# tlroy/thermalporous

Measured on AMD Instinct MI355X. Metric: Newton steps/s, SPE10 60x220x85 two-phase (FGMRES its/s in config), higher is better.
Workload: dtype f64; 1 GPU; BASELINE config 4: two-phase 3D SPE10-like 60x220x85, wells+heaters, pc_cptr, maxdt 0.1 day; grid 60x220x85 (synthetic default_rng(10) field); FGMRES rtol 1e-08; timed at dt = maxdt after an untimed spin-up along the reference's dt ramp; newton_its=84, fgmres_its=2692, failed_solves=0, slabs=none

## Files before the change

thermalporous_amd/csrc/tp_amg.hip:

```cpp
#include "tp_common.hpp"
#include <algorithm>
#include <cstdlib>

namespace tp {

template <class R>
struct StencilT {
    R *base;
    long slot_stride;
    __host__ __device__ const R *slot(int s) const { return base + (long)s * slot_stride; }
};

__device__ __forceinline__ void cell_ijk(const GridDev &g, long tid, int &i0, int &i1, int &i2) {
    const unsigned t = (unsigned)tid, np = (unsigned)g.np, n0 = (unsigned)g.n0;
    const unsigned q2 = t / np, rem = t - q2 * np, q1 = rem / n0;
    i2 = (int)q2;
    i1 = (int)q1;
    i0 = (int)(rem - q1 * n0);
}

template <class R>
__global__ void k_amg_weights(GridDev g, StencilT<R> A, int axis, double omega, R *wm, R *wp, R *invd,
                              unsigned long long *ratio_slots) {
    const long tid = (long)blockIdx.x * blockDim.x + threadIdx.x;
// ... 84 lines not shown
        const double piv = M[(long)p * n + p];
        __syncthreads();
        for (int e = threadIdx.x; e < n; e += blockDim.x) {
            M[(long)p * n + e] /= piv;
            Minv[(long)p * n + e] /= piv;
        }
        __syncthreads();
        for (int e = threadIdx.x; e < n * n; e += blockDim.x) {
            const int r = e / n, q = e % n;
            if (r == p) continue;
            const double fct = M[(long)r * n + p];
            Minv[(long)r * n + q] -= fct * Minv[(long)p * n + q];
            if (q != p) M[(long)r * n + q] -= fct * M[(long)p * n + q];
        }
        __syncthreads();
        for (int r = threadIdx.x; r < n; r += blockDim.x)
            if (r != p) M[(long)r * n + p] = 0.0;
        __syncthreads();
    }
}

template <class R>
__global__ __launch_bounds__(1024) void k_amg_dense_inverse_lds(GridDev g, StencilT<R> A, int n, double *Minv_out) {
    __shared__ double M[64 * 64];
    __shared__ double I[64 * 64];
    __shared__ double col[64];
    const int t = threadIdx.x, T = blockDim.x;
    const long off[7] = {0, -1, 1, -(long)g.n0, (long)g.n0, -g.np, g.np};
    for (int e = t; e < 64 * 64; e += T) { M[e] = 0.0; I[e] = ((e >> 6) == (e & 63)) ? 1.0 : 0.0; }
    __syncthreads();
    for (int r = t; r < n; r += T) {
        const long c = g.np + r;
        int i0, i1, i2;
        cell_ijk(g, r, i0, i1, i2);
        const bool has[7] = {true, i0 > 0, i0 < g.n0 - 1, i1 > 0, i1 < g.n1 - 1, i2 > 0, i2 < g.n2 - 1};
        for (int s = 0; s < 7; ++s)
            if (has[s]) M[r * 64 + (int)(r + off[s])] += (double)A.slot(s)[c];
    }
    __syncthreads();
    for (int p = 0; p < n; ++p) {
        if (t < n) col[t] = M[t * 64 + p];
        __syncthreads();
        const double piv = col[p];
        if (t < n) M[p * 64 + t] /= piv;
        else if (t >= 64 && t < 64 + n) I[p * 64 + (t - 64)] /= piv;
        __syncthreads();
        for (int e = t; e < n * 64; e += T) {
            const int r = e >> 6, q = e & 63;
            if (r == p || q >= n) continue;
            const double fct = col[r];
            I[e] -= fct * I[p * 64 + q];
            M[e] = (q == p) ? 0.0 : M[e] - fct * M[p * 64 + q];
        }
        __syncthreads();
    }
    for (int e = t; e < n * n; e += T) Minv_out[e] = I[(e / n) * 64 + e % n];
}

typedef double mfma_d4 __attribute__((ext_vector_type(4)));
template <class R>
__global__ __launch_bounds__(1024) void k_amg_dense_inverse_mfma(GridDev g, StencilT<R> A, int n, double *Minv_out) {
    extern __shared__ double lds[];
    double *X = lds;
    double *Rb = X + 64 * 128;
    double *Cb = Rb + 4 * 128;
    double *Pi = Cb + 64 * 4;
    const int t = threadIdx.x, T = blockDim.x, lane = t & 63, wave = t >> 6;
    const long off[7] = {0, -1, 1, -(long)g.n0, (long)g.n0, -g.np, g.np};
    for (int e = t; e < 64 * 128; e += T) {
        const int r = e >> 7, q = e & 127;
        X[e] = (q == r + 64 || (q == r && r >= n)) ? 1.0 : 0.0;
    }
    __syncthreads();
    for (int r = t; r < n; r += T) {
        const long c = g.np + r;
        int i0, i1, i2;
        cell_ijk(g, r, i0, i1, i2);
        const bool has[7] = {true, i0 > 0, i0 < g.n0 - 1, i1 > 0, i1 < g.n1 - 1, i2 > 0, i2 < g.n2 - 1};
        for (int s = 0; s < 7; ++s)
            if (has[s]) X[r * 128 + (int)(r + off[s])] += (double)A.slot(s)[c];
    }
    __syncthreads();
    for (int p0 = 0; p0 < 64; p0 += 4) {
        if (t == 0) {
            double P[4][4], Q[4][4];
#pragma unroll
            for (int i = 0; i < 4; ++i)
#pragma unroll
                for (int j = 0; j < 4; ++j) { P[i][j] = X[(p0 + i) * 128 + p0 + j]; Q[i][j] = i == j ? 1.0 : 0.0; }
#pragma unroll
            for (int p = 0; p < 4; ++p) {
                const double ip = 1.0 / P[p][p];
#pragma unroll
                for (int j = 0; j < 4; ++j) { P[p][j] *= ip; Q[p][j] *= ip; }
#pragma unroll
                for (int i = 0; i < 4; ++i) {
                    if (i == p) continue;
                    const double f = P[i][p];
#pragma unroll
                    for (int j = 0; j < 4; ++j) { P[i][j] -= f * P[p][j]; Q[i][j] -= f * Q[p][j]; }
                }
            }
#pragma unroll
            for (int i = 0; i < 4; ++i)
#pragma unroll
                for (int j = 0; j < 4; ++j) Pi[i * 4 + j] = Q[i][j];
        }
        __syncthreads();
        if (t < 512) {
            const int i = t >> 7, q = t & 127;
            double v = 0.0;
#pragma unroll
            for (int m = 0; m < 4; ++m) v += Pi[i * 4 + m] * X[(p0 + m) * 128 + q];
            Rb[i * 128 + q] = v;
        } else if (t < 768) {
            const int r = (t - 512) >> 2, j = t & 3;
            Cb[r * 4 + j] = (r >= p0 && r < p0 + 4) ? 0.0 : X[r * 128 + p0 + j];
        }
        __syncthreads();
#pragma unroll
        for (int h = 0; h < 2; ++h) {
            const int rt = wave >> 2, ct = 2 * (wave & 3) + h;
            const double a = -Cb[(rt * 16 + (lane & 15)) * 4 + (lane >> 4)];
            const double b = Rb[(lane >> 4) * 128 + ct * 16 + (lane & 15)];
            mfma_d4 acc;
            double *xp = X + (rt * 16 + (lane >> 4)) * 128 + ct * 16 + (lane & 15);
#pragma unroll
            for (int q = 0; q < 4; ++q) acc[q] = xp[q * 4 * 128];
            acc = __builtin_amdgcn_mfma_f64_16x16x4f64(a, b, acc, 0, 0, 0);
#pragma unroll
            for (int q = 0; q < 4; ++q) {
                const int row = rt * 16 + (lane >> 4) + 4 * q;
                xp[q * 4 * 128] = (row >= p0 && row < p0 + 4) ? Rb[(row - p0) * 128 + ct * 16 + (lane & 15)] : acc[q];
            }
        }
        __syncthreads();
    }
    for (int e = t; e < n * n; e += T) Minv_out[e] = X[(e / n) * 128 + 64 + e % n];
}

template <class R>
struct LevelDevT {
    GridDev g;
    StencilT<R> op;
    const R *invd, *wm, *wp;
    double *b, *x, *x2, *e;
    int axis;
    int pre, post;
    int pad_;
    double omega;
};

template <class R, bool REG>
__device__ __forceinline__ double invd_at(const LevelDevT<R> &L, long c) {
    if constexpr (REG) return (double)(R)(L.omega / (double)L.op.slot(0)[c]);
    else return (double)L.invd[c];
}

__device__ __forceinline__ void nb_offsets(const GridDev &g, long (&off)[7]) {
    off[0] = 0; off[1] = -1; off[2] = 1; off[3] = -(long)g.n0; off[4] = g.n0; off[5] = -g.np; off[6] = g.np;
}

template <class R, bool REG>
__device__ __forceinline__ double pre2_cell(const LevelDevT<R> &L, const double *__restrict__ b, long tid) {
    const long c = L.g.np + tid;
    long off[7];
    nb_offsets(L.g, off);
    double s = 0.0, ic = 0.0;
#pragma unroll
    for (int k = 0; k < 7; ++k) {
        const long n = c + off[k];
        double iv;
        if constexpr (REG) {
            const double d = (double)L.op.slot(0)[n];
            const double q = (double)(R)(L.omega / d);
            iv = d != 0.0 ? q : 0.0;
        } else {
            iv = (double)L.invd[n];
        }
        if (k == 0) ic = iv;
        s += L.op.slot(k)[c] * (iv * b[n]);
    }
    const double x1 = ic * b[c];
    return x1 + ic * (b[c] - s);
}

template <class R, bool REG = false>
__device__ __forceinline__ double jacobi_cell(const LevelDevT<R> &L, const double *__restrict__ b,
                                              const double *__restrict__ x, long tid) {
    const long c = L.g.np + tid;
    long off[7];
    nb_offsets(L.g, off);
    double s = 0.0;
#pragma unroll
    for (int k = 0; k < 7; ++k) s += L.op.slot(k)[c] * x[c + off[k]];
    return x[c] + invd_at<R, REG>(L, c) * (b[c] - s);
}

template <class R>
__device__ __forceinline__ double resid_at(const LevelDevT<R> &L, const double *__restrict__ b,
                                           const double *__restrict__ x, long c) {
    long off[7];
    nb_offsets(L.g, off);
    double s = 0.0;
#pragma unroll
    for (int k = 0; k < 7; ++k) s += L.op.slot(k)[c] * x[c + off[k]];
    return b[c] - s;
}

template <class R>
__device__ __forceinline__ double resid_restrict_cell(const LevelDevT<R> &Lf, const GridDev &gc,
                                                      const double *__restrict__ b, const double *__restrict__ x,
                                                      long tidc) {
    int I[3];
    cell_ijk(gc, tidc, I[0], I[1], I[2]);
    const int a = Lf.axis;
    int F[3] = {I[0], I[1], I[2]};
    const GridDev &gf = Lf.g;
    F[a] = 2 * I[a] + par_of(gf, a);
    const int nfa = a == 0 ? gf.n0 : (a == 1 ? gf.n1 : gf.n2);
    const long stride = a == 0 ? 1 : (a == 1 ? gf.n0 : gf.np);
    const long f = gf.np + (long)F[0] + (long)gf.n0 * F[1] + gf.np * F[2];
    const bool hm = F[a] - 1 >= 0, hp = F[a] + 1 < nfa;
    const long fm = hm ? f - stride : f, fp = hp ? f + stride : f;
    const double vm = (double)Lf.wp[fm] * resid_at(Lf, b, x, fm), vp = (double)Lf.wm[fp] * resid_at(Lf, b, x, fp);
    return resid_at(Lf, b, x, f) + (hm ? vm : 0.0) + (hp ? vp : 0.0);
}

template <class R>
__device__ __forceinline__ double restrict_cell(const LevelDevT<R> &Lf, const GridDev &gc, const double *__restrict__ r,
                                                long tidc) {
    int I[3];
    cell_ijk(gc, tidc, I[0], I[1], I[2]);
    const int a = Lf.axis;
    int F[3] = {I[0], I[1], I[2]};
    const GridDev &gf = Lf.g;
    F[a] = 2 * I[a] + par_of(gf, a);
    const int nfa = a == 0 ? gf.n0 : (a == 1 ? gf.n1 : gf.n2);
    const long stride = a == 0 ? 1 : (a == 1 ? gf.n0 : gf.np);
    const long f = gf.np + (long)F[0] + (long)gf.n0 * F[1] + gf.np * F[2];
    const bool hm = F[a] - 1 >= 0 || open_lo(gf, a), hp = F[a] + 1 < nfa || open_hi(gf, a);
    const long fm = hm ? f - stride : f, fp = hp ? f + stride : f;
    const double vm = (double)Lf.wp[fm] * r[fm], vp = (double)Lf.wm[fp] * r[fp];
    return r[f] + (hm ? vm : 0.0) + (hp ? vp : 0.0);
}

template <class R, bool MASK = true>
__device__ __forceinline__ double prolong_val(const LevelDevT<R> &Lf, const GridDev &gc, const double *__restrict__ ec,
                                              int F0, int F1, int F2) {
    const GridDev &g = Lf.g;
    const int a = Lf.axis;
    const int p = par_of(g, a);
    const int Fa = a == 0 ? F0 : (a == 1 ? F1 : F2);
    const int Ia = (Fa - p) >> 1;
    const bool isF = (Fa + p) & 1;
    const int I0 = a == 0 ? Ia : F0, I1 = a == 1 ? Ia : F1, I2 = a == 2 ? Ia : F2;
    const long ci = gc.np + (long)I0 + (long)gc.n0 * I1 + gc.np * I2;
    const long cf = g.np + (long)F0 + (long)g.n0 * F1 + g.np * F2;
    const long cs = a == 0 ? 1 : (a == 1 ? gc.n0 : gc.np);
    const int nca = a == 0 ? gc.n0 : (a == 1 ? gc.n1 : gc.n2);
    const bool hasR = isF && (Ia + 1 < nca || open_hi(gc, a));
    const double wm = (double)Lf.wm[cf], wp = (double)Lf.wp[cf];
    const double e0 = ec[ci], e1 = ec[hasR ? ci + cs : ci];
    if constexpr (!MASK) return isF ? wm * e0 + (hasR ? wp * e1 : 0.0) : e0;
    const double fF = isF ? 1.0 : 0.0, fR = hasR ? 1.0 : 0.0;
    return (1.0 - fF) * e0 + fF * (wm * e0 + fR * (wp * e1));
}

template <class R, bool REG = false>
__device__ __forceinline__ double prolong_jacobi_cell(const LevelDevT<R> &Lf, const GridDev &gc,
                                                      const double *__restrict__ b, const double *x,
                                                      const double *__restrict__ ec, long tid) {
    const GridDev &g = Lf.g;
    int i0, i1, i2;
    cell_ijk(g, tid, i0, i1, i2);
    const long c = g.np + tid;
    const int m0 = max(i0 - 1, 0), p0 = min(i0 + 1, g.n0 - 1);
    const int m1 = max(i1 - 1, 0), p1 = min(i1 + 1, g.n1 - 1);
    const int m2 = max(i2 - 1, g.nb_lo ? -1 : 0), p2 = min(i2 + 1, g.nb_hi ? g.n2 : g.n2 - 1);
    double v[7];
    v[0] = prolong_val(Lf, gc, ec, i0, i1, i2);
    v[1] = prolong_val(Lf, gc, ec, m0, i1, i2);
    v[2] = prolong_val(Lf, gc, ec, p0, i1, i2);
    v[3] = prolong_val(Lf, gc, ec, i0, m1, i2);
    v[4] = prolong_val(Lf, gc, ec, i0, p1, i2);
    v[5] = prolong_val(Lf, gc, ec, i0, i1, m2);
    v[6] = prolong_val(Lf, gc, ec, i0, i1, p2);
    if (x) {
        const long cn[7] = {c, c + (m0 - i0), c + (p0 - i0), c + (long)g.n0 * (m1 - i1), c + (long)g.n0 * (p1 - i1),
                            c + g.np * (m2 - i2), c + g.np * (p2 - i2)};
#pragma unroll
        for (int k = 0; k < 7; ++k) v[k] += x[cn[k]];
    }
    double s = 0.0;
#pragma unroll
    for (int k = 0; k < 7; ++k) s += (double)Lf.op.slot(k)[c] * v[k];
    return v[0] + invd_at<R, REG>(Lf, c) * (b[c] - s);
}

template <class R>
__device__ __forceinline__ double restrict_at(const LevelDevT<R> &Lf, const double *__restrict__ r, int I0, int I1, int I2) {
    const GridDev &gf = Lf.g;
    const int a = Lf.axis;
    const int F0 = a == 0 ? 2 * I0 : I0, F1 = a == 1 ? 2 * I1 : I1, F2 = a == 2 ? 2 * I2 : I2;
    const int Fa = a == 0 ? F0 : (a == 1 ? F1 : F2);
    const int nfa = a == 0 ? gf.n0 : (a == 1 ? gf.n1 : gf.n2);
    const long stride = a == 0 ? 1 : (a == 1 ? gf.n0 : gf.np);
    const long f = gf.np + (long)F0 + (long)gf.n0 * F1 + gf.np * F2;
    const bool hm = Fa - 1 >= 0, hp = Fa + 1 < nfa;
    const long fm = hm ? f - stride : f, fp = hp ? f + stride : f;
    const double vm = (double)Lf.wp[fm] * r[fm], vp = (double)Lf.wm[fp] * r[fp];
    return r[f] + (hm ? vm : 0.0) + (hp ? vp : 0.0);
}
template <class R>
__device__ __forceinline__ double restrict2_cell(const LevelDevT<R> &L0, const LevelDevT<R> &L1, const GridDev &g2,
                                                 const double *__restrict__ r, long tid2) {
    int I[3];
    cell_ijk(g2, tid2, I[0], I[1], I[2]);
    const GridDev &g1 = L1.g;
    const int a = L1.axis;
    int M[3] = {I[0], I[1], I[2]};
    M[a] = 2 * I[a];
    const int n1a = a == 0 ? g1.n0 : (a == 1 ? g1.n1 : g1.n2);
    const long stride = a == 0 ? 1 : (a == 1 ? g1.n0 : g1.np);
    const long m = g1.np + (long)M[0] + (long)g1.n0 * M[1] + g1.np * M[2];
    const bool hm = M[a] - 1 >= 0, hp = M[a] + 1 < n1a;
    int Mm[3] = {M[0], M[1], M[2]}, Mp[3] = {M[0], M[1], M[2]};
    Mm[a] -= hm ? 1 : 0;
    Mp[a] += hp ? 1 : 0;
    const double v0 = restrict_at(L0, r, M[0], M[1], M[2]);
    const double vm = (double)L1.wp[hm ? m - stride : m] * restrict_at(L0, r, Mm[0], Mm[1], Mm[2]);
    const double vp = (double)L1.wm[hp ? m + stride : m] * restrict_at(L0, r, Mp[0], Mp[1], Mp[2]);
    return v0 + (hm ? vm : 0.0) + (hp ? vp : 0.0);
}
template <class R>
__device__ __forceinline__ double prolong2_val(const LevelDevT<R> &L0, const LevelDevT<R> &L1, const GridDev &g2,
                                               const double *__restrict__ e2, int F0, int F1, int F2) {
    const GridDev &g = L0.g, &g1 = L1.g;
    const int a = L0.axis;
    const int Fa = a == 0 ? F0 : (a == 1 ? F1 : F2);
    const int Ia = Fa >> 1;
    const bool isF = Fa & 1;
    const int n1a = a == 0 ? g1.n0 : (a == 1 ? g1.n1 : g1.n2);
    const bool hasR = isF && (Ia + 1 < n1a);
    const int I0 = a == 0 ? Ia : F0, I1 = a == 1 ? Ia : F1, I2 = a == 2 ? Ia : F2;
    const int J0 = I0 + (a == 0 && hasR), J1 = I1 + (a == 1 && hasR), J2 = I2 + (a == 2 && hasR);
    const long cf = g.np + (long)F0 + (long)g.n0 * F1 + g.np * F2;
    const double wm = (double)L0.wm[cf], wp = (double)L0.wp[cf];
    const double v0 = prolong_val(L1, g2, e2, I0, I1, I2), v1 = prolong_val(L1, g2, e2, J0, J1, J2);
    const double fF = isF ? 1.0 : 0.0, fR = hasR ? 1.0 : 0.0;
    return (1.0 - fF) * v0 + fF * (wm * v0 + fR * (wp * v1));
}
template <class R, bool REG = false>
__device__ __forceinline__ double prolong2_jacobi_cell(const LevelDevT<R> &L0, const LevelDevT<R> &L1, const GridDev &g2,
                                                       const double *__restrict__ b, const double *__restrict__ e2,
                                                       long tid) {
    const GridDev &g = L0.g;
    int i0, i1, i2;
    cell_ijk(g, tid, i0, i1, i2);
    const long c = g.np + tid;
    const int m0 = max(i0 - 1, 0), p0 = min(i0 + 1, g.n0 - 1);
    const int m1 = max(i1 - 1, 0), p1 = min(i1 + 1, g.n1 - 1);
    const int m2 = max(i2 - 1, 0), p2 = min(i2 + 1, g.n2 - 1);
    double v[7];
    v[0] = prolong2_val(L0, L1, g2, e2, i0, i1, i2);
    v[1] = prolong2_val(L0, L1, g2, e2, m0, i1, i2);
    v[2] = prolong2_val(L0, L1, g2, e2, p0, i1, i2);
    v[3] = prolong2_val(L0, L1, g2, e2, i0, m1, i2);
    v[4] = prolong2_val(L0, L1, g2, e2, i0, p1, i2);
    v[5] = prolong2_val(L0, L1, g2, e2, i0, i1, m2);
    v[6] = prolong2_val(L0, L1, g2, e2, i0, i1, p2);
    double s = 0.0;
#pragma unroll
    for (int k = 0; k < 7; ++k) s += (double)L0.op.slot(k)[c] * v[k];
    return v[0] + invd_at<R, REG>(L0, c) * (b[c] - s);
}

template <class R, bool REG>
__global__ __launch_bounds__(256) void k_amg_pre(LevelDevT<R> L, const double *b, int two, double *out) {
    const long tid = xcd_tid();
    if (tid >= L.g.nown) return;
    const long c = L.g.np + tid;
    out[c] = two ? pre2_cell<R, REG>(L, b, tid) : invd_at<R, REG>(L, c) * b[c];
}
template <class R, bool REG>
__global__ __launch_bounds__(256) void k_amg_jacobi(LevelDevT<R> L, const double *b, const double *x, double *out) {
    const long tid = xcd_tid();
    if (tid >= L.g.nown) return;
    out[L.g.np + tid] = jacobi_cell<R, REG>(L, b, x, tid);
}
template <class R>
__global__ __launch_bounds__(256) void k_amg_resid_restrict(LevelDevT<R> Lf, GridDev gc, const double *b,
                                                            const double *x, double *rc) {
    const long tid = xcd_tid();
    if (tid >= gc.nown) return;
    rc[gc.np + tid] = resid_restrict_cell(Lf, gc, b, x, tid);
}
template <class R, bool REG>
__global__ __launch_bounds__(256) void k_amg_prolong_jacobi(LevelDevT<R> Lf, GridDev gc, const double *b,
                                                            const double *x, const double *ec, double *out) {
    const long tid = xcd_tid();
    if (tid >= Lf.g.nown) return;
    out[Lf.g.np + tid] = prolong_jacobi_cell<R, REG>(Lf, gc, b, x, ec, tid);
}

template <class R>
__global__ __launch_bounds__(256) void k_amg_restrict2(LevelDevT<R> L0, LevelDevT<R> L1, GridDev g2, const double *r,
                                                       double *rc) {
    const long tid = xcd_tid();
    if (tid >= g2.nown) return;
    rc[g2.np + tid] = restrict2_cell(L0, L1, g2, r, tid);
}
template <class R, bool REG>
__global__ __launch_bounds__(256) void k_amg_prolong2_jacobi(LevelDevT<R> L0, LevelDevT<R> L1, GridDev g2, const double *b,
                                                             const double *e2, double *out) {
    const long tid = xcd_tid();
    if (tid >= L0.g.nown) return;
    out[L0.g.np + tid] = prolong2_jacobi_cell<R, REG>(L0, L1, g2, b, e2, tid);
}

template <class R>
__global__ __launch_bounds__(256) void k_amg_resid(LevelDevT<R> L, const double *__restrict__ b,
                                                   const double *__restrict__ x, double *__restrict__ r) {
    const long tid = xcd_tid();
    if (tid >= L.g.nown) return;
    r[L.g.np + tid] = resid_at(L, b, x, L.g.np + tid);
}
template <class R>
__global__ __launch_bounds__(256) void k_amg_restrict(LevelDevT<R> Lf, GridDev gc, const double *__restrict__ r,
                                                      double *__restrict__ rc) {
    const long tid = xcd_tid();
    if (tid >= gc.nown) return;
    rc[gc.np + tid] = restrict_cell(Lf, gc, r, tid);
}
struct RrTile {
    int W, H;
    int nr, nfa;
    unsigned ntw, nta;
    unsigned ntiles;
    long sa, so;
    long csa, cso;
};
template <class R, bool FLAT, int K>
__global__ __launch_bounds__(TP_BLOCK) void k_amg_resid_restrict_tile(LevelDevT<R> Lf, GridDev gc, RrTile T,
                                                                      const double *__restrict__ b,
                                                                      const double *__restrict__ x, double *__restrict__ rc) {
    constexpr int NS = K * TP_BLOCK;
    __shared__ double s_m[NS], s_p[NS];
    const unsigned nb = gridDim.x, bi = blockIdx.x;
    const unsigned tile = (bi & 7u) * (nb >> 3) + (bi >> 3);
    if (tile >= T.ntiles) return;
    const int t = (int)threadIdx.x;
    const GridDev &g = Lf.g;
    double r[K];
    long cc[K];
    bool outc[K], hm[K], hp[K];
    int lm[K], lp[K];
    unsigned tw = 0, ta = 0, to = 0;
    if constexpr (!FLAT) {
        const unsigned rest = tile / T.ntw;
        tw = tile - rest * T.ntw;
        to = rest / T.nta;
        ta = rest - to * T.nta;
    }
#pragma unroll
    for (int j = 0; j < K; ++j) {
        const int s = j * TP_BLOCK + t;
        long c, cw;
        if constexpr (FLAT) {
            const long raw = (long)tile * (TP_BLOCK - 2) - 1 + t;
            const long tid = raw < 0 ? 0 : (raw < g.nown ? raw : g.nown - 1);
            int i0, i1, i2;
            cell_ijk(g, tid, i0, i1, i2);
            c = g.np + tid;
            cc[j] = gc.np + (long)(i0 >> 1) + (long)gc.n0 * i1 + gc.np * i2;
            outc[j] = raw == tid && t >= 1 && t <= TP_BLOCK - 2 && !(i0 & 1);
            hm[j] = i0 - 1 >= 0;
            hp[j] = i0 + 1 < g.n0;
            lm[j] = max(t - 1, 0);
            lp[j] = min(t + 1, TP_BLOCK - 1);
            cw = c;
        } else {
            const int h = (int)((unsigned)s / (unsigned)T.W), w = s - h * T.W;
            const int q = (int)tw * T.W + w, fa = (int)ta * (T.H - 1) - 1 + h;
            const int qc = min(q, T.nr - 1), fc = min(max(fa, 0), T.nfa - 1);
            c = g.np + (long)qc + T.sa * fc + T.so * to;
            cc[j] = gc.np + (long)qc + T.csa * (fc >> 1) + T.cso * to;
            outc[j] = q == qc && fa == fc && h < T.H && (h & 1);
            hm[j] = fa - 1 >= 0;
            hp[j] = fa + 1 < T.nfa;
            lm[j] = s >= T.W ? s - T.W : s;
            lp[j] = s + T.W < NS ? s + T.W : s;
            cw = c + ((h & 1) ? (hp[j] ? T.sa : -T.sa) : 0);
        }
        r[j] = resid_at(Lf, b, x, c);
        s_m[s] = (double)Lf.wp[cw] * r[j];
        s_p[s] = (double)Lf.wm[cw] * r[j];
    }
    __syncthreads();
#pragma unroll
    for (int j = 0; j < K; ++j) {
        const double vm = s_m[lm[j]], vp = s_p[lp[j]];
        if (outc[j]) rc[cc[j]] = r[j] + (hm[j] ? vm : 0.0) + (hp[j] ? vp : 0.0);
    }
}
constexpr int RR_K = 2;
static RrTile rr_tile(const GridDev &gf, const GridDev &gc, int a) {
    RrTile T = {};
    if (a == 0) {
        T.ntiles = (unsigned)((gf.nown + TP_BLOCK - 3) / (TP_BLOCK - 2));
        return T;
    }
    const int NS = RR_K * TP_BLOCK;
    T.nr = a == 1 ? gf.n0 : (int)gf.np;
    T.nfa = a == 1 ? gf.n1 : gf.n2;
    T.sa = a == 1 ? gf.n0 : gf.np;
    T.so = a == 1 ? gf.np : 0;
    T.csa = a == 1 ? gc.n0 : gc.np;
    T.cso = a == 1 ? gc.np : 0;
    T.W = 32;
    if (a == 1) {
        double best = 0.0;
        for (int W = 16; W <= 36; ++W) {
            const int H = (NS / W - 1) | 1;
            const double e = (double)T.nr / ((double)((T.nr + W - 1) / W) * W) * (W * (H - 1));
            if (e > best) { best = e; T.W = W; }
        }
    }
    const long nca = (T.nfa + 1) / 2, per_max = (((NS / T.W - 1) | 1) - 1) / 2;
    T.nta = (unsigned)((nca + per_max - 1) / per_max);
    T.H = 2 * (int)((nca + T.nta - 1) / T.nta) + 1;
    T.ntw = (unsigned)((T.nr + T.W - 1) / T.W);
    T.ntiles = T.ntw * T.nta * (unsigned)(a == 1 ? gf.n2 : 1);
    return T;
}
template <class R>
__global__ __launch_bounds__(256) void k_amg_prolong_set(LevelDevT<R> Lf, GridDev gc, const double *__restrict__ ec,
                                                         double *__restrict__ out) {
    const long tid = xcd_tid();
    if (tid >= Lf.g.nown) return;
    int i0, i1, i2;
    cell_ijk(Lf.g, tid, i0, i1, i2);
    out[Lf.g.np + tid] = prolong_val<R, false>(Lf, gc, ec, i0, i1, i2);
}
template <class R>
__global__ __launch_bounds__(256) void k_amg_prolong_add(LevelDevT<R> Lf, GridDev gc, const double *__restrict__ ec,
                                                         double *x) {
    const long tid = xcd_tid();
    if (tid >= Lf.g.nown) return;
    int i0, i1, i2;
    cell_ijk(Lf.g, tid, i0, i1, i2);
    x[Lf.g.np + tid] += prolong_val<R, false>(Lf, gc, ec, i0, i1, i2);
}

struct LineDev {
    const double *m, *invd, *ap;
    int G, S;
};

template <class R>
__global__ __launch_bounds__(64) void k_amg_line_factor(GridDev g, StencilT<R> A, int G, double *m, double *invd, double *ap) {
    const long nlines = (long)g.n1 * g.n2;
    const long line = (long)blockIdx.x * G + threadIdx.x;
    if ((int)threadIdx.x >= G || line >= nlines) return;
    const int n0 = g.n0;
    const long c = g.np + line * n0;
    long q = (long)blockIdx.x * n0 * G + threadIdx.x;
    double d = (double)A.slot(0)[c];
    m[q] = 0.0;
    invd[q] = 1.0 / d;
    ap[q] = (double)A.slot(2)[c];
    for (int i = 1; i < n0; ++i) {
        q += G;
        const double mi = (double)A.slot(1)[c + i] / d;
        d = (double)A.slot(0)[c + i] - mi * (double)A.slot(2)[c + i - 1];
        m[q] = mi;
        invd[q] = 1.0 / d;
        ap[q] = (double)A.slot(2)[c + i];
    }
}

template <class R, bool ZERO>
__global__ __launch_bounds__(TP_BLOCK) void k_amg_line_sweep(LevelDevT<R> L, LineDev F, double omega, const double *__restrict__ b,
                                                             const double *__restrict__ x, double *__restrict__ out) {
    extern __shared__ double img[];
    const int n0 = L.g.n0, G = F.G, S = F.S, t = threadIdx.x;
    const long nlines = (long)L.g.n1 * L.g.n2, line0 = (long)blockIdx.x * G;
    const int nl = (int)(nlines - line0 < G ? nlines - line0 : G);
    const int ncell = nl * n0;
    const long c0 = L.g.np + line0 * n0;
    for (int idx = t; idx < ncell; idx += TP_BLOCK) {
        const unsigned j = (unsigned)idx / (unsigned)n0, i = (unsigned)idx - j * (unsigned)n0;
        double r;
        if constexpr (ZERO) r = b[c0 + idx];
        else r = resid_at(L, b, x, c0 + idx);
        img[j * S + i] = r;
    }
    __syncthreads();
    if (t < nl) {
        double *y = img + t * S;
        const long q0 = (long)blockIdx.x * n0 * G + t;
        double v = y[0];
#pragma unroll 4
        for (int i = 1; i < n0; ++i) {
            v = y[i] - F.m[q0 + (long)i * G] * v;
            y[i] = v;
        }
        v *= F.invd[q0 + (long)(n0 - 1) * G];
        y[n0 - 1] = v;
#pragma unroll 4
        for (int i = n0 - 2; i >= 0; --i) {
            const long q = q0 + (long)i * G;
            v = (y[i] - F.ap[q] * v) * F.invd[q];
            y[i] = v;
        }
    }
    __syncthreads();
    for (int idx = t; idx < ncell; idx += TP_BLOCK) {
        const unsigned j = (unsigned)idx / (unsigned)n0, i = (unsigned)idx - j * (unsigned)n0;
        const double e = omega * img[j * S + i];
        if constexpr (ZERO) out[c0 + idx] = e;
        else out[c0 + idx] = x[c0 + idx] + e;
    }
}

template <class R>
__global__ __launch_bounds__(TP_BLOCK) void k_amg_gs_half(LevelDevT<R> L, int colour, const double *__restrict__ b,
                                                          const double *__restrict__ x, double *__restrict__ out) {
    const long tid = xcd_tid();
    if (tid >= L.g.nown) return;
    int i0, i1, i2;
    cell_ijk(L.g, tid, i0, i1, i2);
    const long c = L.g.np + tid;
    long off[7];
    nb_offsets(L.g, off);
    const double a0 = (double)L.op.slot(0)[c], xc = x[c];
    double s = a0 * xc;
#pragma unroll
    for (int k = 1; k < 7; ++k) s += (double)L.op.slot(k)[c] * x[c + off[k]];
    const double upd = xc + (b[c] - s) / a0;
    out[c] = (((i0 + i1 + i2) & 1) == colour) ? upd : xc;
}

template <class R>
__global__ __launch_bounds__(TP_BLOCK) void k_amg_gs_first(LevelDevT<R> L, const double *__restrict__ b, double *__restrict__ out) {
    const long tid = xcd_tid();
    if (tid >= L.g.nown) return;
    int i0, i1, i2;
    cell_ijk(L.g, tid, i0, i1, i2);
    const long c = L.g.np + tid;
    long off[7];
    nb_offsets(L.g, off);
    const bool in[7] = {true, i0 > 0, i0 + 1 < L.g.n0, i1 > 0, i1 + 1 < L.g.n1, i2 > 0, i2 + 1 < L.g.n2};
    const double a0 = (double)L.op.slot(0)[c], bc = b[c];
    double s = 0.0;
#pragma unroll
    for (int k = 1; k < 7; ++k) {
        const long n = in[k] ? c + off[k] : c;
        s += (double)L.op.slot(k)[c] * (b[n] / (double)L.op.slot(0)[n]);
    }
    out[c] = (((i0 + i1 + i2) & 1) ? bc - s : bc) / a0;
}

template <class R>
__device__ __forceinline__ void tail_sweeps(const LevelDevT<R> *lv, int l0, int nlev, int trunc, int ncoarse,
                                            const double *Minv, const double *b_top, double *e_top) {
    constexpr int T = 1024;
    const int t = threadIdx.x;
    for (int l = l0; l < nlev - 1; ++l) {
        const LevelDevT<R> L = lv[l];
        const GridDev gc = lv[l + 1].g;
        const double *b = (l == l0) ? b_top : L.b;
        double *rc = lv[l + 1].b;
        if (L.pre == 0) {
            for (long i = t; i < gc.nown; i += T) rc[gc.np + i] = restrict_cell(L, gc, b, i);
            __syncthreads();
            continue;
        }
        double *cur = L.x, *oth = L.x2;
        for (long i = t; i < L.g.nown; i += T)
            cur[L.g.np + i] = L.pre >= 2 ? pre2_cell<R, false>(L, b, i) : L.invd[L.g.np + i] * b[L.g.np + i];
        __syncthreads();
        for (int k = 2; k < L.pre; ++k) {
            for (long i = t; i < L.g.nown; i += T) oth[L.g.np + i] = jacobi_cell(L, b, cur, i);
            __syncthreads();
            double *tmp = cur; cur = oth; oth = tmp;
        }
        for (long i = t; i < gc.nown; i += T) rc[gc.np + i] = resid_restrict_cell(L, gc, b, cur, i);
        __syncthreads();
    }
    {
        const LevelDevT<R> Lc = lv[nlev - 1];
        const double *b = (nlev - 1 == l0) ? b_top : Lc.b;
        double *e = (nlev - 1 == l0) ? e_top : Lc.e;
        if (trunc >= 0) {
            for (long i = t; i < Lc.g.nown; i += T) e[Lc.g.np + i] = pre2_cell<R, false>(Lc, b, i);
            __syncthreads();
        } else {
        const int grp = t >> 4, gl = t & 15;
        for (int r = grp; r < ncoarse; r += T >> 4) {
            double s = 0.0;
            for (int q = gl; q < ncoarse; q += 16) s += Minv[(long)r * ncoarse + q] * b[Lc.g.np + q];
            s += __shfl_xor(s, 8, 64);
            s += __shfl_xor(s, 4, 64);
            s += __shfl_xor(s, 2, 64);
            s += __shfl_xor(s, 1, 64);
            if (gl == 0) e[Lc.g.np + r] = s;
// ... 349 lines not shown
}

static bool tail_dense_needed(const Amg *amg, bool shape_resolved) {
    return amg->tdense_on && shape_resolved && amg->trunc < 0 && amg->tdense_stamp != amg->setup_id;
}

static void tail_dense_build(tp_ctx *c, Amg *amg) {
    if (amg->tail_lds == 0 && !amg->tdense_scratch.p)
        amg->tdense_scratch.alloc((size_t)amg->tdense_groups * 4 * amg->tail_vec);
    const int lt = amg->plan.tail_level, nlev = (int)amg->lv.size(), n = amg->ncoarse;
    TailBuild tb;
    tb.Tm = amg->tdense.p;
    tb.scratch = amg->tdense_scratch.p;
    tb.vec_doubles = (int)amg->tail_vec;
    const size_t lds = (size_t)4 * amg->tail_lds * sizeof(double);
    const double *Minv = amg->coarse_inv.p + (size_t)n * n;
    if (amg->single)
        hipLaunchKernelGGL((k_amg_tail<float, true>), dim3(amg->tdense_groups), dim3(1024), lds, c->stream,
                           (const LevelDevT<float> *)amg->lvdev.p, lt, nlev, -1, n, Minv, (const double *)nullptr,
                           (double *)nullptr, amg->tail_lds, tb);
    else
        hipLaunchKernelGGL((k_amg_tail<double, true>), dim3(amg->tdense_groups), dim3(1024), lds, c->stream,
                           (const LevelDevT<double> *)amg->lvdev.p, lt, nlev, -1, n, Minv, (const double *)nullptr,
                           (double *)nullptr, amg->tail_lds, tb);
    TP_HIP(hipGetLastError());
    amg->tdense_stamp = amg->setup_id;
    amg->tdense_builds++;
}

template <class R>
static void setup_impl(tp_ctx *c, Amg *amg, const Stencil &A0) {
    AmgLevel *L0 = amg->lv[0];
    const int lg = amg->plan.dist_levels;
    amg->omega = c->opt.amg_omega;
    if (sizeof(R) == sizeof(double)) {
        L0->op = A0;
    } else {
        hipLaunchKernelGGL(k_amg_import<R>, grid_for(L0->g.nown), dim3(256), 0, c->stream, L0->g, A0, (R *)L0->A.p);
        L0->op.base = L0->A.p;
        L0->op.slot_stride = L0->g.ntot;
    }
    const int nratio = c->opt.amg_dom_tau > 0.0 ? std::min({c->opt.amg_full_levels, (int)amg->lv.size() - 1, 8}) : 0;
    if (nratio > 0) TP_HIP(hipMemsetAsync(amg->ratio_dev.p, 0, sizeof(double) * 64 * nratio, c->stream));
    for (size_t l = 0; l < amg->lv.size(); ++l) {
        AmgLevel *L = amg->lv[l];
        const StencilT<R> op{(R *)L->op.base, L->op.slot_stride};
        const bool want_ratio = (int)l < nratio;
        hipLaunchKernelGGL(k_amg_weights<R>, grid_for(L->g.nown, want_ratio ? 1024 : 256), dim3(want_ratio ? 1024 : 256), 0, c->stream, L->g, op, L->axis,
                           c->opt.amg_omega, (R *)L->wm.p, (R *)L->wp.p, (R *)L->invd.p,
                           (int)l < nratio ? (unsigned long long *)amg->ratio_dev.p + 64 * l : (unsigned long long *)nullptr);
        if constexpr (sizeof(R) == sizeof(double)) {
            if (amg->plan.lv[l].line_g > 0) {
                const LineDev F = line_of(amg, (int)l);
                hipLaunchKernelGGL(k_amg_line_factor<R>, dim3((unsigned)line_groups(amg->plan.lv[l])), dim3(64), 0, c->stream, L->g, op,
                                   F.G, const_cast<double *>(F.m), const_cast<double *>(F.invd), const_cast<double *>(F.ap));
            }
        }
        if ((int)l < lg) {
            halo_exchange_raw(c, L->g, L->invd.p, 1, 0, sizeof(R));
            halo_exchange_raw(c, L->g, L->wm.p, 1, 0, sizeof(R));
            halo_exchange_raw(c, L->g, L->wp.p, 1, 0, sizeof(R));
            if (L->axis == 2) halo_exchange_raw(c, L->g, L->op.base, 7, (size_t)L->op.slot_stride * sizeof(R), sizeof(R));
        }
        if (L->axis >= 0) {
            AmgLevel *Lc = amg->lv[l + 1];
            const AmgPlan::View cv = amg->plan.coarse_view((int)l, c->grid.rank);
            hipLaunchKernelGGL(k_amg_coarsen<R>, grid_for(cv.g.nown), dim3(256), 0, c->stream, L->g, cv.g, op, L->axis,
                               (const R *)L->wm.p, (const R *)L->wp.p, (R *)Lc->A.p + cv.off, Lc->g.ntot);
            if ((int)l + 1 == lg)
                gather_ranges(c, Lc->A.p, Lc->g.np, amg->plan.ranges[lg], 7, (size_t)Lc->g.ntot * sizeof(R), sizeof(R));
        }
    }
    AmgLevel *Lc = amg->lv.back();
    const int n = amg->ncoarse;
    const StencilT<R> opc{(R *)Lc->op.base, Lc->op.slot_stride};
    if (n <= 64) {
        const bool mfma = !(getenv("TP_AMG_DENSE_MFMA") && atoi(getenv("TP_AMG_DENSE_MFMA")) == 0);
        if (mfma) {
            const int bytes = (64 * 128 + 4 * 128 + 64 * 4 + 16) * (int)sizeof(double);
            TP_HIP(hipFuncSetAttribute(reinterpret_cast<const void *>(&k_amg_dense_inverse_mfma<R>),
                                       hipFuncAttributeMaxDynamicSharedMemorySize, bytes));
            hipLaunchKernelGGL(k_amg_dense_inverse_mfma<R>, dim3(1), dim3(1024), bytes, c->stream, Lc->g, opc, n,
                               amg->coarse_inv.p + (size_t)n * n);
        } else {
            hipLaunchKernelGGL(k_amg_dense_inverse_lds<R>, dim3(1), dim3(1024), 0, c->stream, Lc->g, opc, n,
                               amg->coarse_inv.p + (size_t)n * n);
        }
    }
    else
        hipLaunchKernelGGL(k_amg_dense_inverse<R>, dim3(1), dim3(256), 0, c->stream, Lc->g, opc, n, amg->coarse_inv.p,
                           amg->coarse_inv.p + (size_t)n * n);
    std::vector<LevelDevT<R>> h;
    for (size_t l = 0; l < amg->lv.size(); ++l) h.push_back(dev_of<R>(amg, (int)l));
    amg->lvhost.assign((const char *)h.data(), (const char *)h.data() + h.size() * sizeof(LevelDevT<R>));
    TP_HIP(hipMemcpyAsync(amg->lvdev.p, amg->lvhost.data(), amg->lvhost.size(), hipMemcpyHostToDevice, c->stream));
    if (nratio > 0) {
        if (lg > 0) allreduce_max(c, amg->ratio_dev.p, 64 * nratio);
        TP_HIP(hipMemcpyAsync(amg->ratio_host, amg->ratio_dev.p, sizeof(double) * 64 * nratio, hipMemcpyDeviceToHost, c->stream));
        TP_HIP(hipEventRecord(amg->ev_ratio, c->stream));
        amg->ratio_pending = true;
    } else if (amg->trunc != -1) {
        amg->trunc = -1;
        c->graph_epoch++;
    }
    amg->setup_id++;
    const bool dense_env = !(getenv("TP_AMG_TAIL_DENSE") && atoi(getenv("TP_AMG_TAIL_DENSE")) == 0);
    const bool dense = dense_env && amg->tdense_eligible && amg->plan.tail_level >= nratio;
    if (dense != amg->tdense_on) {
        amg->tdense_on = dense;
        c->graph_epoch++;
    }
    if (tail_dense_needed(amg, nratio == 0 || amg->setup_id > 1)) tail_dense_build(c, amg);
    TP_HIP(hipGetLastError());
}

bool amg_resolve_trunc(tp_ctx *c, Amg *amg) {
    if (!amg || !amg->ratio_pending) return false;
    TP_HIP(hipEventSynchronize(amg->ev_ratio));
    amg->ratio_pending = false;
    const int nratio = std::min({c->opt.amg_full_levels, (int)amg->lv.size() - 1, 8});
    int t = -1;
    for (int l = 0; l < nratio; ++l) {
        double r = 0.0;
        for (int q = 0; q < 64; ++q) r = std::max(r, amg->ratio_host[64 * l + q]);
        if (l == 0) amg->ratio0 = r;
        if (r <= c->opt.amg_dom_tau) { t = l; break; }
    }
    const bool changed = t != amg->trunc;
    amg->trunc = t;
    if (tail_dense_needed(amg, true)) tail_dense_build(c, amg);
    return changed;
}

void amg_setup(tp_ctx *c, Amg *amg, const Stencil &A0) {
    static_assert(sizeof(LevelDevT<float>) == sizeof(LevelDevT<double>), "descriptor size");
    if (amg->single) setup_impl<float>(c, amg, A0);
    else setup_impl<double>(c, amg, A0);
}

template <class R>
static void vcycle_impl(tp_ctx *c, Amg *amg, const double *b, double *x) {
    const int nlev = (int)amg->lv.size(), lt = amg->plan.tail_level, lg = amg->plan.dist_levels;
    const int trunc = amg->trunc;
    const int ltop = (trunc >= 0 && trunc < lt) ? trunc : lt;
    const dim3 bl(256);
    std::vector<double *> xs(nlev, nullptr);
    static const bool pair_on = !(getenv("TP_AMG_PAIR") && atoi(getenv("TP_AMG_PAIR")) == 0);
    static const bool invd_reg = !(getenv("TP_AMG_INVD_LOAD") && atoi(getenv("TP_AMG_INVD_LOAD")) != 0);
    static const bool rr_fuse = !(getenv("TP_AMG_RR_FUSE") && atoi(getenv("TP_AMG_RR_FUSE")) == 0);
#define TP_AMG_REG_LAUNCH(KERNEL, ...)                                                                         \
    do {                                                                                                       \
        if (invd_reg) hipLaunchKernelGGL((KERNEL<R, true>), __VA_ARGS__);                                      \
        else hipLaunchKernelGGL((KERNEL<R, false>), __VA_ARGS__);                                              \
    } while (0)
    auto paired = [&](int l) {
        if (!pair_on || l < lg || l + 2 > lt || amg->lv[l]->g.nown >= amg->fuse_below) return false;
        if (trunc >= 0 && l + 2 > trunc) return false;
        const AmgPlan::Level &A = amg->plan.lv[l], &B = amg->plan.lv[l + 1];
        return A.pre == 0 && A.post >= 1 && B.pre == 0 && B.post == 0;
    };
    auto hx = [&](int l, const double *v) {
        if (l < lg) halo_exchange(c, amg->lv[l]->g, const_cast<double *>(v), 1, 0);
    };
    auto is_line = [&](int l) { return amg->plan.lv[l].line_g > 0; };
    auto line_sweep = [&](int l, const double *bb, const double *xin, double *xout) {
        if constexpr (sizeof(R) == sizeof(double)) {
            const AmgPlan::Level &P = amg->plan.lv[l];
            const LineDev F = line_of(amg, l);
            const dim3 gl((unsigned)line_groups(P));
            const size_t lds = (size_t)F.G * F.S * sizeof(double);
            if (xin) hipLaunchKernelGGL((k_amg_line_sweep<R, false>), gl, dim3(TP_BLOCK), lds, c->stream, dev_of<R>(amg, l), F, c->opt.amg_omega, bb, xin, xout);
            else hipLaunchKernelGGL((k_amg_line_sweep<R, true>), gl, dim3(TP_BLOCK), lds, c->stream, dev_of<R>(amg, l), F, c->opt.amg_omega, bb, xin, xout);
        } else {
            throw Error("line relaxation (amg_line_levels) with fp32 operators (amg_single)");
        }
    };
    auto is_gs = [&](int l) { return amg->plan.lv[l].gs > 0; };
    auto gs_half = [&](int l, int colour, const double *bb, const double *xin, double *xout) {
        hipLaunchKernelGGL(k_amg_gs_half<R>, xcd_grid(amg->lv[l]->g.nown), bl, 0, c->stream, dev_of<R>(amg, l), colour, bb, xin, xout);
    };
    auto gs_forward = [&](int l, const double *bb) {
        AmgLevel *L = amg->lv[l];
        double *cur = L->x.p, *oth = L->x2.p;
        hipLaunchKernelGGL(k_amg_gs_first<R>, xcd_grid(L->g.nown), bl, 0, c->stream, dev_of<R>(amg, l), bb, cur);
        for (int h = 2; h < 2 * amg->plan.lv[l].gs; ++h) {
            gs_half(l, h & 1, bb, cur, oth);
            std::swap(cur, oth);
        }
        return cur;
    };
    auto gs_backward = [&](int l, const double *bb, double *src, double *out) {
        AmgLevel *L = amg->lv[l];
        const int nh = 2 * amg->plan.lv[l].gs;
        for (int h = 0; h < nh; ++h) {
            double *dst = (h == nh - 1) ? out : (src == L->x.p ? L->x2.p : L->x.p);
            gs_half(l, 1 - (h & 1), bb, src, dst);
            src = dst;
        }
    };
    for (int l = 0; l < ltop; ++l) {
        AmgLevel *L = amg->lv[l];
        AmgLevel *Lc = amg->lv[l + 1];
        const LevelDevT<R> Ld = dev_of<R>(amg, l);
        const AmgPlan::View cv = amg->plan.coarse_view(l, c->grid.rank);
        const double *bl_ = (l == 0) ? b : L->b.p;
        double *bc = Lc->b.p + cv.off;
        const dim3 gr = xcd_grid(L->g.nown);
        const bool slab_axis = l < lg && L->axis == 2;
        if (paired(l)) {
            AmgLevel *L2 = amg->lv[l + 2];
            hipLaunchKernelGGL(k_amg_restrict2<R>, xcd_grid(L2->g.nown), bl, 0, c->stream, Ld,
                               dev_of<R>(amg, l + 1), L2->g, bl_, L2->b.p);
            ++l;
            continue;
        }
        if (Ld.pre == 0) {
            if (slab_axis) hx(l, bl_);
            hipLaunchKernelGGL(k_amg_restrict<R>, xcd_grid(cv.g.nown), bl, 0, c->stream, Ld, cv.g, bl_, bc);
        } else {
            double *cur = L->x.p, *oth = L->x2.p;
            if (is_gs(l)) {
                cur = gs_forward(l, bl_);
                oth = (cur == L->x.p) ? L->x2.p : L->x.p;
            } else if (is_line(l)) {
                line_sweep(l, bl_, nullptr, cur);
                for (int k = 1; k < Ld.pre; ++k) {
                    line_sweep(l, bl_, cur, oth);
                    std::swap(cur, oth);
                }
            } else {
            if (Ld.pre >= 2) hx(l, bl_);
            if (invd_reg && l >= lg) hipLaunchKernelGGL((k_amg_pre<R, true>), gr, bl, 0, c->stream, Ld, bl_, Ld.pre >= 2 ? 1 : 0, cur);
            else hipLaunchKernelGGL((k_amg_pre<R, false>), gr, bl, 0, c->stream, Ld, bl_, Ld.pre >= 2 ? 1 : 0, cur);
            for (int k = 2; k < Ld.pre; ++k) {
                hx(l, cur);
                TP_AMG_REG_LAUNCH(k_amg_jacobi, gr, bl, 0, c->stream, Ld, bl_, (const double *)cur, oth);
                std::swap(cur, oth);
            }
            }
            xs[l] = cur;
            hx(l, cur);
            if (rr_fuse && !slab_axis && L->g.nown >= amg->fuse_below) {
                const RrTile T = rr_tile(L->g, cv.g, L->axis);
                const dim3 gt((T.ntiles + 7u) / 8u * 8u);
                if (L->axis == 0) hipLaunchKernelGGL((k_amg_resid_restrict_tile<R, true, 1>), gt, dim3(TP_BLOCK), 0, c->stream, Ld, cv.g, T, bl_, (const double *)cur, bc);
                else hipLaunchKernelGGL((k_amg_resid_restrict_tile<R, false, RR_K>), gt, dim3(TP_BLOCK), 0, c->stream, Ld, cv.g, T, bl_, (const double *)cur, bc);
            } else if (slab_axis || L->g.nown >= amg->fuse_below) {
                hipLaunchKernelGGL(k_amg_resid<R>, gr, bl, 0, c->stream, Ld, bl_, (const double *)cur, oth);
                if (slab_axis) hx(l, oth);
                hipLaunchKernelGGL(k_amg_restrict<R>, xcd_grid(cv.g.nown), bl, 0, c->stream, Ld, cv.g, (const double *)oth, bc);
            } else {
                hipLaunchKernelGGL(k_amg_resid_restrict<R>, xcd_grid(cv.g.nown), bl, 0, c->stream, Ld, cv.g, bl_,
                                   (const double *)cur, bc);
            }
        }
        if (l + 1 == lg)
            gather_ranges(c, Lc->b.p, Lc->g.np, amg->plan.ranges[lg], 1, 0, sizeof(double));
    }
    if (trunc >= 0 && trunc < lt) {
        AmgLevel *L = amg->lv[trunc];
        const double *bt = (trunc == 0) ? b : L->b.p;
        double *et = (trunc == 0) ? x : L->e.p;
        if (is_gs(trunc)) {
            gs_backward(trunc, bt, gs_forward(trunc, bt), et);
        } else if (is_line(trunc)) {
            line_sweep(trunc, bt, nullptr, L->x.p);
            line_sweep(trunc, bt, L->x.p, et);
        } else {
        hx(trunc, bt);
        if (invd_reg && trunc >= lg) hipLaunchKernelGGL((k_amg_pre<R, true>), xcd_grid(L->g.nown), bl, 0, c->stream, dev_of<R>(amg, trunc), bt, 1, et);
        else hipLaunchKernelGGL((k_amg_pre<R, false>), xcd_grid(L->g.nown), bl, 0, c->stream, dev_of<R>(amg, trunc), bt, 1, et);
        }
    } else {
        AmgLevel *Lt = amg->lv[lt];
        const double *bt = (lt == 0) ? b : Lt->b.p;
        double *et = (lt == 0) ? x : Lt->e.p;
        const int n = amg->ncoarse;
        if (amg->tdense_on) {
            TP_REQUIRE(trunc < 0 && amg->tdense_stamp == amg->setup_id, "the dense AMG tail was not formed for the last set-up");
            const int nt = (int)Lt->g.nown;
            const dim3 gd((unsigned)((nt + TP_BLOCK / 64 - 1) / (TP_BLOCK / 64))), bd(TP_BLOCK);
            const double *Tm = amg->tdense.p;
            if (nt <= 256) hipLaunchKernelGGL(k_amg_tail_dense<4>, gd, bd, 0, c->stream, Tm, nt, Lt->g.np, bt, et);
            else if (nt <= 512) hipLaunchKernelGGL(k_amg_tail_dense<8>, gd, bd, 0, c->stream, Tm, nt, Lt->g.np, bt, et);
            else if (nt <= 768) hipLaunchKernelGGL(k_amg_tail_dense<12>, gd, bd, 0, c->stream, Tm, nt, Lt->g.np, bt, et);
            else hipLaunchKernelGGL(k_amg_tail_dense<16>, gd, bd, 0, c->stream, Tm, nt, Lt->g.np, bt, et);
            amg->tdense_applies++;
        } else {
            hipLaunchKernelGGL((k_amg_tail<R, false>), dim3(1), dim3(1024), (size_t)4 * amg->tail_lds * sizeof(double), c->stream,
                               (const LevelDevT<R> *)amg->lvdev.p, lt, nlev, trunc, n,
                               (const double *)(amg->coarse_inv.p + (size_t)n * n), bt, et, amg->tail_lds, TailBuild());
            amg->tail_launches++;
        }
    }
    for (int l = ltop - 1; l >= 0; --l) {
        AmgLevel *L = amg->lv[l];
        AmgLevel *Lc = amg->lv[l + 1];
        const LevelDevT<R> Ld = dev_of<R>(amg, l);
        const AmgPlan::View cv = amg->plan.coarse_view(l, c->grid.rank);
        const double *bl_ = (l == 0) ? b : L->b.p;
        double *out = (l == 0) ? x : L->e.p;
        const double *ec = Lc->e.p + cv.off;
        const dim3 gr = xcd_grid(L->g.nown);
        double *src = xs[l];
        double *dst = (Ld.post == 1) ? out : (src == L->x.p ? L->x2.p : L->x.p);
        if (l >= 1 && paired(l - 1)) continue;
        if (paired(l)) {
            AmgLevel *L2 = amg->lv[l + 2];
            TP_AMG_REG_LAUNCH(k_amg_prolong2_jacobi, gr, bl, 0, c->stream, Ld, dev_of<R>(amg, l + 1), L2->g, bl_,
                               (const double *)L2->e.p, dst);
            for (int k = 1; k < Ld.post; ++k) {
                src = dst;
                dst = (k == Ld.post - 1) ? out : (src == L->x.p ? L->x2.p : L->x.p);
                TP_AMG_REG_LAUNCH(k_amg_jacobi, gr, bl, 0, c->stream, Ld, bl_, (const double *)src, dst);
            }
            continue;
        }
        hx(l + 1, Lc->e.p);
        if (Ld.post == 0) {
            hipLaunchKernelGGL(k_amg_prolong_set<R>, gr, bl, 0, c->stream, Ld, cv.g, ec, out);
            continue;
        }
        if (is_gs(l)) {
            TP_REQUIRE(src, "a Gauss-Seidel level has pre-smoothing sweeps");
            hipLaunchKernelGGL(k_amg_prolong_add<R>, gr, bl, 0, c->stream, Ld, cv.g, ec, src);
            gs_backward(l, bl_, src, out);
            continue;
        }
        if (is_line(l)) {
            TP_REQUIRE(src, "a line level has pre-smoothing sweeps");
            hipLaunchKernelGGL(k_amg_prolong_add<R>, gr, bl, 0, c->stream, Ld, cv.g, ec, src);
            line_sweep(l, bl_, src, dst);
            for (int k = 1; k < Ld.post; ++k) {
                src = dst;
                dst = (k == Ld.post - 1) ? out : (src == L->x.p ? L->x2.p : L->x.p);
                line_sweep(l, bl_, src, dst);
            }
            continue;
        }
        if (src && L->g.nown >= amg->fuse_below) {
            hipLaunchKernelGGL(k_amg_prolong_add<R>, gr, bl, 0, c->stream, Ld, cv.g, ec, src);
            hx(l, src);
            TP_AMG_REG_LAUNCH(k_amg_jacobi, gr, bl, 0, c->stream, Ld, bl_, (const double *)src, dst);
        } else {
            TP_AMG_REG_LAUNCH(k_amg_prolong_jacobi, gr, bl, 0, c->stream, Ld, cv.g, bl_, (const double *)src, ec, dst);
        }
        for (int k = 1; k < Ld.post; ++k) {
            src = dst;
            dst = (k == Ld.post - 1) ? out : (src == L->x.p ? L->x2.p : L->x.p);
            hx(l, src);
            TP_AMG_REG_LAUNCH(k_amg_jacobi, gr, bl, 0, c->stream, Ld, bl_, (const double *)src, dst);
        }
    }
#undef TP_AMG_REG_LAUNCH
    TP_HIP(hipGetLastError());
}

void amg_vcycle(tp_ctx *c, Amg *amg, const double *b, double *x) {
    TP_REQUIRE(amg && !amg->lv.empty(), "AMG not set up");
    TP_REQUIRE(!amg->ratio_pending, "amg_resolve_trunc must run after a set-up and before the first cycle");
    TP_REQUIRE(x != amg->lv[0]->x.p && x != amg->lv[0]->x2.p && b != x, "aliasing in amg_vcycle");
    if (amg->single) vcycle_impl<float>(c, amg, b, x);
    else vcycle_impl<double>(c, amg, b, x);
}

}
```

Measured before the change: 30.14 Newton steps/s.

## Fuse AMG prolongation-add with first post-smoothing Jacobi sweep using LDS tiles

On large non-distributed AMG levels, the separate prolong_add kernel followed by a Jacobi sweep is replaced by one tiled kernel. Each block works on one z-plane run, computes prolongated-plus-current values for its cells and the n0-wide halo rows into shared memory, then applies the 7-point Jacobi update. This removes a kernel launch and a full write/read of the corrected fine-level vector. The cost is redundant prolongation work for halo rows and z neighbours, and the fused path does not write the corrected vector back to src.

Measured after the change: 30.63 Newton steps/s, median of 6. 1.02x the previous value.

```diff
diff --git a/thermalporous_amd/csrc/tp_amg.hip b/thermalporous_amd/csrc/tp_amg.hip
--- a/thermalporous_amd/csrc/tp_amg.hip
+++ b/thermalporous_amd/csrc/tp_amg.hip
@@ -260,9 +260,13 @@
 };
 
 template <class R, bool REG>
+__device__ __forceinline__ double invd_from(const LevelDevT<R> &L, R s) {
+    if constexpr (REG) return (double)(R)(L.omega / (double)s);
+    else return (double)s;
+}
+template <class R, bool REG>
 __device__ __forceinline__ double invd_at(const LevelDevT<R> &L, long c) {
-    if constexpr (REG) return (double)(R)(L.omega / (double)L.op.slot(0)[c]);
-    else return (double)L.invd[c];
+    return invd_from<R, REG>(L, REG ? L.op.slot(0)[c] : L.invd[c]);
 }
 
 __device__ __forceinline__ void nb_offsets(const GridDev &g, long (&off)[7]) {
@@ -293,16 +297,25 @@
     return x1 + ic * (b[c] - s);
 }
 
+template <class R>
+__device__ __forceinline__ double jacobi_update(const R (&a)[7], const double (&v)[7], double iv, double bc) {
+    double s = 0.0;
+#pragma unroll
+    for (int k = 0; k < 7; ++k) s += a[k] * v[k];
+    return v[0] + iv * (bc - s);
+}
+
 template <class R, bool REG = false>
 __device__ __forceinline__ double jacobi_cell(const LevelDevT<R> &L, const double *__restrict__ b,
                                               const double *__restrict__ x, long tid) {
     const long c = L.g.np + tid;
     long off[7];
     nb_offsets(L.g, off);
-    double s = 0.0;
-#pragma unroll
-    for (int k = 0; k < 7; ++k) s += L.op.slot(k)[c] * x[c + off[k]];
-    return x[c] + invd_at<R, REG>(L, c) * (b[c] - s);
+    R a[7];
+    double v[7];
+#pragma unroll
+    for (int k = 0; k < 7; ++k) { a[k] = L.op.slot(k)[c]; v[k] = x[c + off[k]]; }
+    return jacobi_update<R>(a, v, invd_at<R, REG>(L, c), b[c]);
 }
 
 template <class R>
@@ -373,6 +386,12 @@
     if constexpr (!MASK) return isF ? wm * e0 + (hasR ? wp * e1 : 0.0) : e0;
     const double fF = isF ? 1.0 : 0.0, fR = hasR ? 1.0 : 0.0;
     return (1.0 - fF) * e0 + fF * (wm * e0 + fR * (wp * e1));
+}
+
+template <class R>
+__device__ __forceinline__ double prolong_added(const LevelDevT<R> &Lf, const GridDev &gc, const double *__restrict__ ec,
+                                                const double *x, int F0, int F1, int F2) {
+    return x[Lf.g.np + (long)F0 + (long)Lf.g.n0 * F1 + Lf.g.np * F2] + prolong_val<R, false>(Lf, gc, ec, F0, F1, F2);
 }
 
 template <class R, bool REG = false>
@@ -658,9 +677,50 @@
     if (tid >= Lf.g.nown) return;
     int i0, i1, i2;
     cell_ijk(Lf.g, tid, i0, i1, i2);
-    x[Lf.g.np + tid] += prolong_val<R, false>(Lf, gc, ec, i0, i1, i2);
-}
-
+    x[Lf.g.np + tid] = prolong_added<R>(Lf, gc, ec, x, i0, i1, i2);
+}
+
+constexpr int PJ_NH_MAX = 4;
+template <class R, bool REG, int NH>
+__global__ __launch_bounds__(TP_BLOCK) void k_amg_prolong_jacobi_tile(LevelDevT<R> Lf, GridDev gc, unsigned nruns, unsigned ntiles,
+                                                                      const double *__restrict__ b,
+                                                                      const double *__restrict__ x,
+                                                                      const double *__restrict__ ec, double *__restrict__ out) {
+    __shared__ double s_x[(NH + 1) * TP_BLOCK];
+    const unsigned nb = gridDim.x, bi = blockIdx.x;
+    const unsigned tile = (bi & 7u) * (nb >> 3) + (bi >> 3);
+    if (tile >= ntiles) return;
+    const int t = (int)threadIdx.x;
+    const GridDev &g = Lf.g;
+    const int n0 = g.n0, npl = (int)g.np;
+    const int k = (int)(tile / nruns);
+    const int q0 = (int)(tile - (unsigned)k * nruns) * TP_BLOCK;
+    const int q = q0 + t, qc = min(q, npl - 1);
+    const int i1 = (int)((unsigned)qc / (unsigned)n0), i0 = qc - i1 * n0;
+    const long c = g.np + (long)qc + g.np * k;
+    const double xm = prolong_added<R>(Lf, gc, ec, x, i0, i1, max(k - 1, 0));
+    const double xc = prolong_added<R>(Lf, gc, ec, x, i0, i1, k);
+    R a[7];
+#pragma unroll
+    for (int s = 0; s < 7; ++s) a[s] = Lf.op.slot(s)[c];
+    const R ivs = REG ? a[0] : Lf.invd[c];
+    const double bc = b[c];
+    const double xp = prolong_added<R>(Lf, gc, ec, x, i0, i1, min(k + 1, g.n2 - 1));
+    s_x[n0 + t] = xc;
+#pragma unroll
+    for (int m = 0; m < NH; ++m) {
+        const int h = m * TP_BLOCK + t;
+        const int r = h < n0 ? h : h + TP_BLOCK;
+        const int qh = min(max(q0 - n0 + r, 0), npl - 1);
+        const int h1 = (int)((unsigned)qh / (unsigned)n0);
+        const double xh = prolong_added<R>(Lf, gc, ec, x, qh - h1 * n0, h1, k);
+        if (h < 2 * n0) s_x[r] = xh;
+    }
+    __syncthreads();
+    const double v[7] = {xc, s_x[n0 + t - 1], s_x[n0 + t + 1], s_x[t], s_x[2 * n0 + t], xm, xp};
+    const double y = jacobi_update<R>(a, v, invd_from<R, REG>(Lf, ivs), bc);
+    if (q < npl) out[c] = y;
+}
 struct LineDev {
     const double *m, *invd, *ap;
     int G, S;
@@ -1316,6 +1376,12 @@
     do {                                                                                                       \
         if (invd_reg) hipLaunchKernelGGL((KERNEL<R, true>), __VA_ARGS__);                                      \
         else hipLaunchKernelGGL((KERNEL<R, false>), __VA_ARGS__);                                              \
+    } while (0)
+    static const bool pj_fuse = !(getenv("TP_AMG_PJ_FUSE") && atoi(getenv("TP_AMG_PJ_FUSE")) == 0);
+#define TP_AMG_PJ_LAUNCH(NH)                                                                                                           \
+    do {                                                                                                                       \
+        if (invd_reg) hipLaunchKernelGGL((k_amg_prolong_jacobi_tile<R, true, NH>), gt, dim3(TP_BLOCK), 0, c->stream, Ld, cv.g, nruns, ntiles, bl_, (const double *)src, ec, dst); \
+        else hipLaunchKernelGGL((k_amg_prolong_jacobi_tile<R, false, NH>), gt, dim3(TP_BLOCK), 0, c->stream, Ld, cv.g, nruns, ntiles, bl_, (const double *)src, ec, dst); \
     } while (0)
     auto paired = [&](int l) {
         if (!pair_on || l < lg || l + 2 > lt || amg->lv[l]->g.nown >= amg->fuse_below) return false;
@@ -1502,7 +1568,12 @@
             }
             continue;
         }
-        if (src && L->g.nown >= amg->fuse_below) {
+        if (pj_fuse && l >= lg && src && L->g.nown >= amg->fuse_below && 2 * L->g.n0 <= PJ_NH_MAX * TP_BLOCK) {
+            const unsigned nruns = (unsigned)((L->g.np + TP_BLOCK - 1) / TP_BLOCK), ntiles = nruns * (unsigned)L->g.n2;
+            const dim3 gt((ntiles + 7u) / 8u * 8u);
+            if (2 * L->g.n0 <= TP_BLOCK) TP_AMG_PJ_LAUNCH(1);
+            else TP_AMG_PJ_LAUNCH(PJ_NH_MAX);
+        } else if (src && L->g.nown >= amg->fuse_below) {
             hipLaunchKernelGGL(k_amg_prolong_add<R>, gr, bl, 0, c->stream, Ld, cv.g, ec, src);
             hx(l, src);
             TP_AMG_REG_LAUNCH(k_amg_jacobi, gr, bl, 0, c->stream, Ld, bl_, (const double *)src, dst);
@@ -1516,6 +1587,7 @@
             TP_AMG_REG_LAUNCH(k_amg_jacobi, gr, bl, 0, c->stream, Ld, bl_, (const double *)src, dst);
         }
     }
+#undef TP_AMG_PJ_LAUNCH
 #undef TP_AMG_REG_LAUNCH
     TP_HIP(hipGetLastError());
 }
```
